# yangdongchao/Text-to-sound-Synthesis

Hardware: AMD Instinct MI355X
Metric: 10s clips/sec whole-node, 100-step Diffsound sample + VQ decode + vocoder (higher is better)
Workload: dtype f32 via 2-way fp16 split (3 MFMA passes, fp32 accumulate); 1 GPU; BASELINE configs[2]: full pipeline, batch 64 per GPU, 100 diffusion steps, codebook 256: CLIP text tower -> 19-layer denoiser -> SpecVQGAN decode -> MelGAN 22 kHz; global_batch=64, n_layer=19, parallelism=caption-sharded x1

## Files before the change

include/diffsound_hip.h:

```cpp
#ifndef DIFFSOUND_HIP_H
#define DIFFSOUND_HIP_H
#include <stdint.h>
#ifdef __cplusplus
extern "C" {
#endif

typedef void* ds_stream_t;

int ds_version(void);
const char* ds_last_error_string(void);

enum { DS_LOAD_DENSE = 0, DS_LOAD_CONV2D = 1, DS_LOAD_CONV1D = 2, DS_LOAD_CONVT1D = 3 };
enum { DS_PRO_NONE = 0, DS_PRO_AFFINE = 1, DS_PRO_AFFINE_SWISH = 2, DS_PRO_LRELU = 3 };
enum { DS_ACT_NONE = 0, DS_ACT_GELU2 = 1, DS_ACT_TANH = 2 };
enum { DS_STORE_ROW = 0, DS_STORE_BATCH_T = 1, DS_STORE_CONVT = 2, DS_STORE_ATTN = 3 };

typedef struct ds_gemm_desc {
    const float* A;
    const float* W;
    const float* bias;
    const float* R;
    float* C;
    int32_t M, N, K;
    int32_t lda, ldw, ldc, ldr;
    int32_t groups;
    int64_t a_gstride, w_gstride, c_gstride;
    int32_t loader, pro, act, store;
    const float* pro_scale;
    const float* pro_shift;
    int32_t rows_per_sample;
    int32_t Cin;
    int32_t H, Wd;
    int32_t up;
    int32_t taps, dil;
    int32_t ct_r, ct_p, ct_tin;
    int32_t f16_round;
    int64_t w3_plane;
    float out_scale;
    int32_t a_split, c_split;
    int64_t a_plane, c_plane;
    void* attn_kv;
    int32_t attn_heads, attn_nkey;
    int64_t attn_qplane;
} ds_gemm_desc;

int ds_gemm(const ds_gemm_desc* d, ds_stream_t stream);
void ds_gemm_force_tile(int cfg);
int ds_gemm_f16x2(const ds_gemm_desc* d, ds_stream_t stream);
int ds_gemm_f16x2_multi(const ds_gemm_desc* descs, int n, int cfg, ds_stream_t stream);
int ds_conv2d_f16x2(const ds_gemm_desc* d, ds_stream_t stream);
void ds_gemm_f16x2_force_tile(int cfg);
int ds_gemm_f16x2_auto_tile(int M, int N, int groups);
void ds_gemm_f16x2_set_balance_slots(int slots);
int ds_gemm_f16x2_plan(int cfg, int M, int N, int store, int* m_off, int* nbig, int* nsmall);

int ds_embed(const int64_t* tokens, const float* emb, const float* pos, float* out, int M, int L, int D,
             ds_stream_t stream);
int ds_adaln(const float* x, float* y, int M, int L, int D, const float* table, const int64_t* t,
             ds_stream_t stream);
int ds_layernorm(const float* x, float* y, int M, int D, const float* gamma, const float* beta,
                 ds_stream_t stream);
int ds_attention(const float* q, int ldq, const float* k, int ldk, const float* v, int ldv, float* o, int ldo,
                 int B, int heads, int Lq, int Lk, float scale, ds_stream_t stream);

int ds_attention_ex(const float* q, int ldq, const float* k, int ldk, const float* v, int ldv, float* o, int ldo,
                    int B, int heads, int Lq, int Lk, float scale, int causal, int f16_round, ds_stream_t stream);
int ds_attention_f16x2(const float* q, int ldq, const float* k, int ldk, const float* v, int ldv, float* o, int ldo,
                       int B, int heads, int Lq, int Lk, float scale, ds_stream_t stream);
int ds_adaln_split(const float* x, void* yh, int M, int L, int D, const float* table, const int64_t* t,
                   ds_stream_t stream);
int ds_layernorm_split(const float* x, void* yh, int M, int D, const float* gamma, const float* beta,
                       ds_stream_t stream);
int ds_attention_f16x2_split(const float* q, int ldq, const float* k, int ldk, const float* v, int ldv, void* oh,
                             int ldo, int B, int heads, int Lq, int Lk, float scale, ds_stream_t stream);
int ds_attn_nkey(int Lk);
int ds_attention_f16x2_ready(const void* qh, long long q_plane, const void* kv_img, void* oh, int ldo, int B, int heads,
                             int Lq, int Lk, float scale, ds_stream_t stream);
int ds_attn_pack_kv(const float* kv, int ld, int v_col, void* img, int B, int heads, int Lk, ds_stream_t stream);
int ds_embed_f16(const int64_t* tokens, const float* emb, const float* pos, float* out, int M, int L, int D,
                 ds_stream_t stream);
int ds_layernorm_f16(const float* x, float* y, int M, int D, const float* gamma, const float* beta,
                     ds_stream_t stream);
int ds_l2norm_rows_f16(const float* x, float* y, int M, int D, ds_stream_t stream);

// ... 243 lines not shown
```

text-to-sound-synthesis_amd/_lib.py:

```python
import ctypes as C
import os

import torch

_HERE = os.path.dirname(os.path.abspath(__file__))
LIB_PATH = os.environ.get("DIFFSOUND_LIB") or os.path.join(_HERE, "libdiffsound_hip.so")

LOAD_DENSE, LOAD_CONV2D, LOAD_CONV1D, LOAD_CONVT1D = 0, 1, 2, 3
PRO_NONE, PRO_AFFINE, PRO_AFFINE_SWISH, PRO_LRELU = 0, 1, 2, 3
ACT_NONE, ACT_GELU2, ACT_TANH = 0, 1, 2
STORE_ROW, STORE_BATCH_T, STORE_CONVT, STORE_ATTN = 0, 1, 2, 3
(LP_ADALN1, LP_W_QKV, LP_B_QKV, LP_W_PROJ1, LP_B_PROJ1, LP_ADALN2, LP_W_Q2, LP_B_Q2, LP_W_KV2, LP_B_KV2,
 LP_W_PROJ2, LP_B_PROJ2, LP_LN2_G, LP_LN2_B, LP_W_FC1, LP_B_FC1, LP_W_FC2, LP_B_FC2, LP_COUNT) = range(19)

_vp, _i32, _i64, _f = C.c_void_p, C.c_int32, C.c_int64, C.c_float


class GemmDesc(C.Structure):
    _fields_ = [("A", _vp), ("W", _vp), ("bias", _vp), ("R", _vp), ("C", _vp),
                ("M", _i32), ("N", _i32), ("K", _i32),
                ("lda", _i32), ("ldw", _i32), ("ldc", _i32), ("ldr", _i32),
                ("groups", _i32),
                ("a_gstride", _i64), ("w_gstride", _i64), ("c_gstride", _i64),
                ("loader", _i32), ("pro", _i32), ("act", _i32), ("store", _i32),
                ("pro_scale", _vp), ("pro_shift", _vp),
                ("rows_per_sample", _i32), ("Cin", _i32), ("H", _i32), ("Wd", _i32), ("up", _i32),
                ("taps", _i32), ("dil", _i32), ("ct_r", _i32), ("ct_p", _i32), ("ct_tin", _i32),
                ("f16_round", _i32), ("w3_plane", _i64), ("out_scale", _f),
                ("a_split", _i32), ("c_split", _i32), ("a_plane", _i64), ("c_plane", _i64),
                ("attn_kv", _vp), ("attn_heads", _i32), ("attn_nkey", _i32), ("attn_qplane", _i64)]


class DenoiserDesc(C.Structure):
    _fields_ = [("n_layer", _i32), ("n_embd", _i32), ("n_head", _i32), ("seq_len", _i32),
                ("cond_len", _i32), ("cond_dim", _i32), ("n_codes", _i32), ("n_steps", _i32),
                ("mlp_mult", _i32),
                ("tok_emb", _vp), ("pos_emb", _vp), ("lnf_g", _vp), ("lnf_b", _vp),
                ("w_logits", _vp), ("b_logits", _vp), ("sched", _vp)]


_PROTOS = {
    "ds_version": (C.c_int, []),
    "ds_last_error_string": (C.c_char_p, []),
    "ds_gemm": (C.c_int, [C.POINTER(GemmDesc), _vp]),
    "ds_gemm_force_tile": (None, [C.c_int]),
    "ds_gemm_f16x2": (C.c_int, [C.POINTER(GemmDesc), _vp]),
    "ds_conv2d_f16x2": (C.c_int, [C.POINTER(GemmDesc), _vp]),
    "ds_gemm_f16x2_multi": (C.c_int, [C.POINTER(GemmDesc), C.c_int, C.c_int, _vp]),
    "ds_gemm_f16x2_auto_tile": (C.c_int, [C.c_int, C.c_int, C.c_int]),
    "ds_gemm_f16x2_force_tile": (None, [C.c_int]),
    "ds_gemm_f16x2_set_balance_slots": (None, [C.c_int]),
    "ds_gemm_f16x2_plan": (C.c_int, [C.c_int, C.c_int, C.c_int, C.c_int, C.POINTER(C.c_int), C.POINTER(C.c_int), C.POINTER(C.c_int)]),
    "ds_denoiser_set_split_weights": (C.c_int, [_vp, C.c_int, C.POINTER(_vp), C.POINTER(_f), _vp, _f]),
    "ds_embed": (C.c_int, [_vp, _vp, _vp, _vp, C.c_int, C.c_int, C.c_int, _vp]),
    "ds_adaln": (C.c_int, [_vp, _vp, C.c_int, C.c_int, C.c_int, _vp, _vp, _vp]),
    "ds_layernorm": (C.c_int, [_vp, _vp, C.c_int, C.c_int, _vp, _vp, _vp]),
    "ds_attention": (C.c_int, [_vp, C.c_int, _vp, C.c_int, _vp, C.c_int, _vp, C.c_int,
                               C.c_int, C.c_int, C.c_int, C.c_int, _f, _vp]),
    "ds_attention_ex": (C.c_int, [_vp, C.c_int, _vp, C.c_int, _vp, C.c_int, _vp, C.c_int,
                                  C.c_int, C.c_int, C.c_int, C.c_int, _f, C.c_int, C.c_int, _vp]),
    "ds_attention_f16x2": (C.c_int, [_vp, C.c_int, _vp, C.c_int, _vp, C.c_int, _vp, C.c_int,
                                     C.c_int, C.c_int, C.c_int, C.c_int, _f, _vp]),
    "ds_adaln_split": (C.c_int, [_vp, _vp, C.c_int, C.c_int, C.c_int, _vp, _vp, _vp]),
    "ds_layernorm_split": (C.c_int, [_vp, _vp, C.c_int, C.c_int, _vp, _vp, _vp]),
    "ds_attention_f16x2_split": (C.c_int, [_vp, C.c_int, _vp, C.c_int, _vp, C.c_int, _vp, C.c_int,
                                           C.c_int, C.c_int, C.c_int, C.c_int, _f, _vp]),
    "ds_attn_nkey": (C.c_int, [C.c_int]),
    "ds_attention_f16x2_ready": (C.c_int, [_vp, _i64, _vp, _vp, C.c_int, C.c_int, C.c_int, C.c_int, C.c_int, _f, _vp]),
    "ds_attn_pack_kv": (C.c_int, [_vp, C.c_int, C.c_int, _vp, C.c_int, C.c_int, C.c_int, _vp]),
    "ds_embed_f16": (C.c_int, [_vp, _vp, _vp, _vp, C.c_int, C.c_int, C.c_int, _vp]),
    "ds_layernorm_f16": (C.c_int, [_vp, _vp, C.c_int, C.c_int, _vp, _vp, _vp]),
    "ds_l2norm_rows_f16": (C.c_int, [_vp, _vp, C.c_int, C.c_int, _vp]),
    "ds_sample_tail": (C.c_int, [_vp, _vp, _vp, _vp, _vp, _vp, _vp, _vp, _vp,
                                 C.c_int, C.c_int, C.c_int, C.c_int, C.c_int, _f, _vp]),
    "ds_sample_tail_ex": (C.c_int, [_vp, _vp, _vp, _vp, _vp, _vp, _vp, _vp, _vp,
                                    C.c_int, C.c_int, C.c_int, C.c_int, C.c_int, _f, C.c_int, _vp]),
    "ds_q_sample": (C.c_int, [_vp, _vp, _vp, _vp, _vp, C.c_int, C.c_int, C.c_int, C.c_int, _vp]),
    "ds_philox_uniforms": (C.c_int, [_vp, C.c_uint64, C.c_int, C.c_int, _vp, C.c_int, C.c_int, C.c_int, _vp]),
    "ds_sample_tail_rng": (C.c_int, [_vp, _vp, _vp, _vp, C.c_uint64, C.c_int, _vp, _vp, C.c_int, C.c_int, C.c_int, C.c_int,
                                     C.c_int, _f, C.c_int, _vp]),
    "ds_q_sample_rng": (C.c_int, [_vp, _vp, _vp, C.c_uint64, C.c_int, _vp, _vp, C.c_int, C.c_int, C.c_int, C.c_int, _vp]),
    "ds_vq_argmin": (C.c_int, [_vp, _vp, _vp, _vp, _vp, C.c_int, C.c_int, C.c_int, _vp]),
    "ds_loss_tail": (C.c_int, [_vp, _vp, _vp, _vp, _vp, _vp, _vp, _vp, _vp, C.c_int, C.c_int, C.c_int, C.c_int, _vp]),
# ... 258 lines not shown
```

text-to-sound-synthesis_amd/csrc/gemm_f16x2_ps.hip:

```cpp
#include <stdlib.h>

#include "common.h"


typedef _Float16 h8 __attribute__((ext_vector_type(8)));
typedef unsigned u32x4 __attribute__((ext_vector_type(4)));
typedef unsigned u32x2 __attribute__((ext_vector_type(2)));
typedef __attribute__((address_space(1))) const void* ds_gptr;
typedef __attribute__((address_space(3))) void* ds_lptr;

#define PS_HLD 32
#define PS_BM 288
#define PS_BN 256
#define PS_LEAD 6
#define PS_GM 4
#define PS_STAGE_BYTES (2 * 2 * (PS_BM + PS_BN) * PS_HLD * 2)
#define PS_EPI_BYTES (2 * 64 * (PS_BN + 4) * 4)
#ifndef PS_DIRECT_SPLIT
#define PS_DIRECT_SPLIT 1
#endif
#ifndef PS_DIRECT_QK
#define PS_DIRECT_QK 0
#endif
#define PS_LDS_BYTES (PS_EPI_BYTES > PS_STAGE_BYTES ? PS_EPI_BYTES : PS_STAGE_BYTES)
#define PS_SIG(q_) ((0x78 >> (2 * (q_))) & 3)

enum { PS_EPI_ROW = 0, PS_EPI_SPLIT = 1, PS_EPI_ATTN = 2 };

template <int EPI, bool NB16>
__global__ __launch_bounds__(512, 1) void ds_gemm_f16x2_ps_kernel(const GemmParams p) {
    extern __shared__ __attribute__((aligned(16))) unsigned char smem_raw[];
    constexpr int BM = PS_BM, BN = PS_BN, HLD = PS_HLD, LEAD = PS_LEAD;
    constexpr int APL = BM * HLD, BPL = BN * HLD, STAGE = 2 * (APL + BPL);
    _Float16* smem = (_Float16*)smem_raw;
    const int tid = threadIdx.x, lane = tid & 63, wave = tid >> 6, l31 = lane & 31, hh = lane >> 5;
    const int wr = wave >> 2, wc = wave & 3;
    const int L = p.rows_per_sample;
    const int tiles_n = p.N / BN, nblk = gridDim.x;
    int bid = blockIdx.x;
    {
        const int xcd = bid & 7, idx = bid >> 3, q = nblk >> 3, r = nblk & 7;
        bid = (xcd < r ? xcd * (q + 1) : r * (q + 1) + (xcd - r) * q) + idx;
    }
    int tm_, tn_;
    {
        const int tiles_m = p.M / L;
        const int per = PS_GM * tiles_n, grp = bid / per, first = grp * PS_GM;
        const int gsz = tiles_m - first < PS_GM ? tiles_m - first : PS_GM;
        const int in = bid - grp * per;
        tm_ = first + in % gsz;
        tn_ = in / gsz;
    }
    const int row_lo = tm_ * L;
    const int m0 = (row_lo >> 4) << 4, n0 = tn_ * BN;
    const int nk = p.K / 32;
    const _Float16* Ap = (const _Float16*)p.A;
    const _Float16* Wp = (const _Float16*)p.W;
    unsigned long long src[4][2], src8;
    int ldsoff[4][2], ldsoff8;
    const unsigned lane16 = lane * 16;
    const int rgsA = (p.M + 15) >> 4, rgsB = (p.N + 15) >> 4;
#define PS_BASE(dst_, ptr_)                                                                          \
    do {                                                                                             \
        const unsigned long long a_ = (unsigned long long)(ptr_);                                    \
        dst_ = ((unsigned long long)(unsigned)__builtin_amdgcn_readfirstlane((unsigned)(a_ >> 32)) << 32) | \
               (unsigned long long)(unsigned)__builtin_amdgcn_readfirstlane((unsigned)a_);           \
    } while (0)
#pragma unroll
    for (int ty = 0; ty < 4; ++ty)
#pragma unroll
        for (int k = 0; k < 2; ++k) {
            const int idx = 2 * wave + k, plane = idx >> 3, r = idx & 7;
            const bool isA = (ty == 0 || ty == 3);
            const int s = isA ? (ty == 3) : (ty == 2);
            const int gip = isA ? (r >> 2) * 8 + s * 4 + (r & 3)
                                : (r >> 1) * 4 + s * 2 + (r & 1);
            int rg = ((isA ? m0 : n0) >> 4) + gip;
            const int rgs = isA ? rgsA : rgsB;
            if (rg >= rgs) rg = rgs - 1;
            PS_BASE(src[ty][k], (isA ? Ap + plane * p.a_plane : Wp + plane * p.w3_plane) + (size_t)rg * nk * 512);
            ldsoff[ty][k] = __builtin_amdgcn_readfirstlane((isA ? plane * 18 + gip : 36 + plane * 16 + gip) * 1024);
        }
    {
        const int e = wave & 3, plane = e >> 1, gip = 16 + (e & 1);
        int rg = (m0 >> 4) + gip;
        if (rg >= rgsA) rg = rgsA - 1;
        PS_BASE(src8, Ap + plane * p.a_plane + (size_t)rg * nk * 512);
        ldsoff8 = __builtin_amdgcn_readfirstlane((plane * 18 + gip) * 1024);
    }
#define PS_ISSUE(tile_, ty_, buf_)                                                                   \
    do {                                                                                             \
        _Pragma("unroll") for (int k = 0; k < 2; ++k)                                                \
            __builtin_amdgcn_global_load_lds((ds_gptr)((const unsigned char*)(src[ty_][k] + (unsigned long long)(tile_) * 1024) + lane16), \
                                             (ds_lptr)(smem_raw + (buf_) * (STAGE * 2) + ldsoff[ty_][k]), 16, 0, 0); \
        if ((ty_) == 3)                                                                              \
            __builtin_amdgcn_global_load_lds((ds_gptr)((const unsigned char*)(src8 + (unsigned long long)(tile_) * 1024) + lane16), \
                                             (ds_lptr)(smem_raw + (buf_) * (STAGE * 2) + ldsoff8), 16, 0, 0); \
    } while (0)
#define PS_DMA_ASM(base_, lds_, stage_)                                                              \
    do {                                                                                             \
        asm volatile("s_add_u32 m0, %2, %3\n\ts_nop 0\n\tglobal_load_lds_dwordx4 %0, %1"            \
                     :: "v"(lane16), "s"(base_), "s"(lds_), "n"(stage_) : "memory", "scc", "m0");    \
        base_ += 1024;                                                                               \
    } while (0)
#define PS_ISSUE_LOOP(tq_, ty_, buf_)                                                                \
    do {                                                                                             \
        PS_DMA_ASM(cur[ty_][0], ldsabs[ty_][0], (buf_) * (STAGE * 2));                               \
        PS_DMA_ASM(cur[ty_][1], ldsabs[ty_][1], (buf_) * (STAGE * 2));                               \
        if ((ty_) == 3) PS_DMA_ASM(cur8, ldsabs8, (buf_) * (STAGE * 2));                             \
    } while (0)
#define PS_FENCE()                                                                                   \
    do { asm volatile("" ::: "memory"); __builtin_amdgcn_sched_barrier(0); } while (0)
#define PS_BAR()                                                                                     \
    do { PS_FENCE(); __builtin_amdgcn_s_barrier(); PS_FENCE(); } while (0)
#define PS_LBAR() PS_BAR()
    const int swz[2] = {((0 + hh) ^ ((l31 >> 2) & 3)) * 8, ((2 + hh) ^ ((l31 >> 2) & 3)) * 8};
    f32x16 acc[4][2], acc8;
    f32x4 acc9[2];
#pragma unroll
    for (int r = 0; r < 16; ++r) acc8[r] = 0.f;
#pragma unroll
    for (int tt = 0; tt < 2; ++tt) acc9[tt] = f32x4{0.f, 0.f, 0.f, 0.f};
#pragma unroll
    for (int i = 0; i < 4; ++i)
#pragma unroll
        for (int j = 0; j < 2; ++j)
#pragma unroll
            for (int r = 0; r < 16; ++r) acc[i][j][r] = 0.f;
    h8 a0[2][2], a1[2][2];
    h8 b0[2][2], b1[2][2];
    h8 e0[2], e1[2];
    h8 ea0, ea1, eb0[2], eb1[2];
    const int l15 = PS_SIG((lane >> 2) & 3) * 4 + (lane & 3);
    const int swzq = ((lane >> 4) ^ ((l15 >> 2) & 3)) * 8;
#define PS_READ_A(buf_, s_)                                                                          \
    do {                                                                                             \
        const _Float16* Ac = smem + (buf_) * STAGE + (wr * 128 + (s_) * 64 + l31) * HLD;             \
        _Pragma("unroll") for (int ks = 0; ks < 2; ++ks)                                             \
            _Pragma("unroll") for (int ib = 0; ib < 2; ++ib) {                                       \
                a0[ks][ib] = *(const h8*)(Ac + ib * 32 * HLD + swz[ks]);                             \
                a1[ks][ib] = *(const h8*)(Ac + APL + ib * 32 * HLD + swz[ks]);                       \
            }                                                                                        \
    } while (0)
#define PS_READ_E(buf_)                                                                              \
    do {                                                                                             \
        const _Float16* Ec = smem + (buf_) * STAGE + (256 + l31) * HLD;                              \
        _Pragma("unroll") for (int ks = 0; ks < 2; ++ks) {                                           \
            e0[ks] = *(const h8*)(Ec + swz[ks]);                                                     \
            e1[ks] = *(const h8*)(Ec + APL + swz[ks]);                                               \
        }                                                                                            \
    } while (0)
#define PS_READ_B(buf_, s_)                                                                          \
    do {                                                                                             \
        const _Float16* Bc = smem + (buf_) * STAGE + 2 * APL + (wc * 64 + (s_) * 32 + l31) * HLD;    \
        _Pragma("unroll") for (int ks = 0; ks < 2; ++ks) {                                           \
            b0[s_][ks] = *(const h8*)(Bc + swz[ks]);                                                 \
            b1[s_][ks] = *(const h8*)(Bc + BPL + swz[ks]);                                           \
        }                                                                                            \
    } while (0)
#define PS_QUAD(sa_, sb_)                                                                            \
    do {                                                                                             \
        _Pragma("unroll") for (int ks = 0; ks < 2; ++ks) {                                           \
            _Pragma("unroll") for (int ib = 0; ib < 2; ++ib)                                         \
                acc[2 * (sa_) + ib][sb_] = __builtin_amdgcn_mfma_f32_32x32x16_f16(b0[sb_][ks], a1[ks][ib], acc[2 * (sa_) + ib][sb_], 0, 0, 0); \
            _Pragma("unroll") for (int ib = 0; ib < 2; ++ib)                                         \
                acc[2 * (sa_) + ib][sb_] = __builtin_amdgcn_mfma_f32_32x32x16_f16(b1[sb_][ks], a0[ks][ib], acc[2 * (sa_) + ib][sb_], 0, 0, 0); \
            _Pragma("unroll") for (int ib = 0; ib < 2; ++ib)                                         \
                acc[2 * (sa_) + ib][sb_] = __builtin_amdgcn_mfma_f32_32x32x16_f16(b0[sb_][ks], a0[ks][ib], acc[2 * (sa_) + ib][sb_], 0, 0, 0); \
        }                                                                                            \
    } while (0)
#define PS_EXTRA(sb_)                                                                                \
    do {                                                                                             \
        _Pragma("unroll") for (int ks = 0; ks < 2; ++ks) {                                           \
            acc8 = __builtin_amdgcn_mfma_f32_32x32x16_f16(b0[sb_][ks], e1[ks], acc8, 0, 0, 0);       \
            acc8 = __builtin_amdgcn_mfma_f32_32x32x16_f16(b1[sb_][ks], e0[ks], acc8, 0, 0, 0);       \
            acc8 = __builtin_amdgcn_mfma_f32_32x32x16_f16(b0[sb_][ks], e0[ks], acc8, 0, 0, 0);       \
        }                                                                                            \
    } while (0)
#define PS_READ_EB16(buf_)                                                                           \
    do {                                                                                             \
        const _Float16* Bc = smem + (buf_) * STAGE + 2 * APL + ((2 * wc + wr) * 32 + l15) * HLD;     \
        _Pragma("unroll") for (int tt = 0; tt < 2; ++tt) {                                           \
            eb0[tt] = *(const h8*)(Bc + tt * 16 * HLD + swzq);                                       \
            eb1[tt] = *(const h8*)(Bc + BPL + tt * 16 * HLD + swzq);                                 \
        }                                                                                            \
    } while (0)
#define PS_READ_EA16(buf_)                                                                           \
    do {                                                                                             \
        const _Float16* Ec = smem + (buf_) * STAGE + (256 + l15) * HLD;                              \
        ea0 = *(const h8*)(Ec + swzq);                                                               \
        ea1 = *(const h8*)(Ec + APL + swzq);                                                         \
    } while (0)
#define PS_EXTRA16()                                                                                 \
    do {                                                                                             \
        _Pragma("unroll") for (int tt = 0; tt < 2; ++tt) {                                           \
            acc9[tt] = __builtin_amdgcn_mfma_f32_16x16x32_f16(eb0[tt], ea1, acc9[tt], 0, 0, 0);      \
            acc9[tt] = __builtin_amdgcn_mfma_f32_16x16x32_f16(eb1[tt], ea0, acc9[tt], 0, 0, 0);      \
            acc9[tt] = __builtin_amdgcn_mfma_f32_16x16x32_f16(eb0[tt], ea0, acc9[tt], 0, 0, 0);      \
        }                                                                                            \
    } while (0)
#define PS_PHASE(P, BUF)                                                                             \
    do {                                                                                             \
        if (P == 0) { PS_READ_A(BUF, 0); PS_READ_B(BUF, 0); }                                        \
        if (P == 1) { PS_READ_B(BUF, 1); if (NB16) PS_READ_EB16(BUF); }                              \
        if (P == 2) { PS_READ_A(BUF, 1); if (NB16) PS_READ_EA16(BUF); }                              \
        if (P == 3 && !NB16) PS_READ_E(BUF);                                                         \
        PS_FENCE();                                                                                  \
        {                                                                                            \
            constexpr int dq = (P) + LEAD;                                     \
            const int tq = t + (dq >> 2);                                                            \
            if (tq < nk) {                                                                           \
                PS_ISSUE_LOOP(tq, dq & 3, ((BUF) + (dq >> 2)) & 1);                                  \
                asm volatile("s_waitcnt vmcnt(9)" ::: "memory");    \
            } else {                                                                                 \
                asm volatile("s_waitcnt vmcnt(0)" ::: "memory");    \
            }                                                                                        \
        }                                                                                            \
        PS_LBAR();                                                                                   \
        __builtin_amdgcn_s_setprio(1);                                                               \
        if (P == 0) PS_QUAD(0, 0);                                                                   \
        if (P == 1) PS_QUAD(0, 1);                                                                   \
        if (P == 2) { PS_QUAD(1, 1); if (NB16) PS_EXTRA16(); }                                       \
        if (P == 3) { PS_QUAD(1, 0); if (!NB16) { if (wr == 0) PS_EXTRA(0); else PS_EXTRA(1); } }    \
        __builtin_amdgcn_s_setprio(0);                                                               \
        PS_LBAR();                                                                                   \
    } while (0)
#pragma unroll
    for (int q = 0; q < LEAD; ++q)
        if ((q >> 2) < nk) PS_ISSUE(q >> 2, q & 3, (q >> 2) & 1);
    if (4 * nk >= LEAD) asm volatile("s_waitcnt vmcnt(9)" ::: "memory");
    else asm volatile("s_waitcnt vmcnt(0)" ::: "memory");
    PS_BAR();
    if (wr == 1) PS_LBAR();
    unsigned long long cur[4][2], cur8 = src8 + 1024;
#pragma unroll
    for (int ty = 0; ty < 4; ++ty) {
        cur[ty][0] = src[ty][0] + (ty < 2 ? 2048 : 1024);
        cur[ty][1] = src[ty][1] + (ty < 2 ? 2048 : 1024);
    }
    const unsigned lds0 = __builtin_amdgcn_readfirstlane((unsigned)(size_t)(__attribute__((address_space(3))) unsigned char*)smem_raw);
    unsigned ldsabs[4][2], ldsabs8 = lds0 + ldsoff8;
#pragma unroll
    for (int ty = 0; ty < 4; ++ty) { ldsabs[ty][0] = lds0 + ldsoff[ty][0]; ldsabs[ty][1] = lds0 + ldsoff[ty][1]; }
    for (int t = 0; t < nk; t += 2) {
        PS_PHASE(0, 0); PS_PHASE(1, 0); PS_PHASE(2, 0); PS_PHASE(3, 0);
        ++t;
        PS_PHASE(0, 1); PS_PHASE(1, 1); PS_PHASE(2, 1); PS_PHASE(3, 1);
        --t;
    }
    if (wr == 0) PS_LBAR();
    asm volatile("s_waitcnt vmcnt(0)" ::: "memory");

    constexpr int WROW = 128, EROW0 = 256;
    constexpr bool HALF_TILE = false;
    const bool hasE = true;
    const int pos0 = 0, tile_rows = L;
#include "gemm_f16x2_ps_epilogue.inc"
}

#define PH_AROWS 144
#define PH_STAGE_BYTES (2 * (PH_AROWS + PS_BN) * PS_HLD * 2)
#define PH_LDS_BYTES (3 * PH_STAGE_BYTES > PS_EPI_BYTES ? 3 * PH_STAGE_BYTES : PS_EPI_BYTES)

template <int EPI>
__global__ __launch_bounds__(512, 1) void ds_gemm_f16x2_ph_kernel(const GemmParams p) {
    extern __shared__ __attribute__((aligned(16))) unsigned char smem_raw[];
    constexpr bool NB16 = true;
    constexpr int BN = PS_BN, HLD = PS_HLD;
    constexpr int APL = PH_AROWS * HLD, BPL = BN * HLD, STAGE = 2 * (APL + BPL);
    _Float16* smem = (_Float16*)smem_raw;
    const int tid = threadIdx.x, lane = tid & 63, wave = tid >> 6, l31 = lane & 31, hh = lane >> 5;
    const int wr = wave >> 2, wc = wave & 3;
    const int L = p.rows_per_sample;
    const int tiles_n = p.N / BN, nblk = gridDim.x;
    int bid = blockIdx.x;
    {
        const int xcd = bid & 7, idx = bid >> 3, q = nblk >> 3, r = nblk & 7;
        bid = (xcd < r ? xcd * (q + 1) : r * (q + 1) + (xcd - r) * q) + idx;
    }
    int th_, tn_;
    {
        const int tiles_m = 2 * (p.M / L);
        const int per = PS_GM * tiles_n, grp = bid / per, first = grp * PS_GM;
        const int gsz = tiles_m - first < PS_GM ? tiles_m - first : PS_GM;
        const int in = bid - grp * per;
        th_ = first + in % gsz;
        tn_ = in / gsz;
    }
    const int tm_ = th_ >> 1;
    const bool hasE = (th_ & 1) == 0;
// ... 135 lines not shown
        else { PH_QUAD(1); if (hasE) PH_EXTRA16(); }                                                 \
        __builtin_amdgcn_s_setprio(0);                                                               \
        PS_BAR();                                                                                    \
    } while (0)
    unsigned long long curA[2] = {srcA[0] + 2048, srcA[1] + 2048}, curE = srcE + 2048;
    unsigned long long curB[2][2] = {{srcB[0][0] + 2048, srcB[0][1] + 2048}, {srcB[1][0] + 2048, srcB[1][1] + 2048}};
    const unsigned lds0 = __builtin_amdgcn_readfirstlane((unsigned)(size_t)(__attribute__((address_space(3))) unsigned char*)smem_raw);
    const unsigned absA[2] = {lds0 + offA[0], lds0 + offA[1]}, absE = lds0 + offE;
    const unsigned absB[2][2] = {{lds0 + offB[0][0], lds0 + offB[0][1]}, {lds0 + offB[1][0], lds0 + offB[1][1]}};
#define PH_ISSUE_LOOP(half_, st_)                                                                    \
    do {                                                                                             \
        if ((half_) == 0) {                                                                          \
            PS_DMA_ASM(curA[0], absA[0], (st_) * (STAGE * 2)); PS_DMA_ASM(curA[1], absA[1], (st_) * (STAGE * 2)); \
            PS_DMA_ASM(curB[0][0], absB[0][0], (st_) * (STAGE * 2)); PS_DMA_ASM(curB[0][1], absB[0][1], (st_) * (STAGE * 2)); \
        } else {                                                                                     \
            PS_DMA_ASM(curB[1][0], absB[1][0], (st_) * (STAGE * 2)); PS_DMA_ASM(curB[1][1], absB[1][1], (st_) * (STAGE * 2)); \
            PS_DMA_ASM(curE, absE, (st_) * (STAGE * 2));                                             \
        }                                                                                            \
    } while (0)
    PH_ISSUE(0, 0, 0); PH_ISSUE(0, 1, 0);
    if (nk > 1) { PH_ISSUE(1, 0, 1); PH_ISSUE(1, 1, 1); asm volatile("s_waitcnt vmcnt(10)" ::: "memory"); }
    else asm volatile("s_waitcnt vmcnt(0)" ::: "memory");
    PS_BAR();
    if (wr == 1) PS_BAR();
    for (int t = 0; t < nk; t += 3) {
        { const int tt = t; PH_PHASE(0, 0); PH_PHASE(1, 0); }
        if (t + 1 < nk) { const int tt = t + 1; PH_PHASE(0, 1); PH_PHASE(1, 1); }
        if (t + 2 < nk) { const int tt = t + 2; PH_PHASE(0, 2); PH_PHASE(1, 2); }
    }
    if (wr == 0) PS_BAR();
    asm volatile("s_waitcnt vmcnt(0)" ::: "memory");
    constexpr int WROW = 64, EROW0 = 128;
    constexpr bool HALF_TILE = true;
#include "gemm_f16x2_ps_epilogue.inc"
}

static bool ps_serves(const GemmParams& p, bool half) {
    const int L = p.rows_per_sample;
    if (!p.a_split || L <= 0 || L > PS_BM - 15 || L <= 240 || p.M % L != 0) return false;
    if (half && L != PS_BM - 16) return false;
    if (p.N % PS_BN != 0 || p.K % 64 != 0 || p.lda != p.K || p.ldw != p.K) return false;
    if (((uintptr_t)p.bias & 15) != 0) return false;
    if (p.store == DS_STORE_ROW && !p.c_split) {
        if (((p.N | p.ldc | p.ldr) & 3) != 0 || (((uintptr_t)p.C | (uintptr_t)p.R) & 15) != 0) return false;
    } else if (p.store == DS_STORE_ROW) {
        if (p.R) return false;
    } else if (p.store == DS_STORE_ATTN) {
        if (p.row_off != 0 || p.attn_heads * 64 % PS_BN != 0) return false;
    } else {
        return false;
    }
    return true;
}

int ds_gemm_f16x2_ps_choice(long B, long N, bool half_ok) {
    const long tf = B * (N / PS_BN), th = 2 * tf;
    const double ef = (double)tf / (double)(((tf + 255) / 256) * 256);
    const double eh = half_ok ? 0.92 * (double)th / (double)(((th + 255) / 256) * 256) : 0.0;
    if (ef < 0.65 && eh < 0.65) return 0;
    return ef >= eh ? 1 : 2;
}

bool ds_gemm_f16x2_ps_applies(const GemmParams& p, bool need_full_grid) {
    if (!ps_serves(p, false)) return false;
    return !need_full_grid || ds_gemm_f16x2_ps_choice(p.M / p.rows_per_sample, p.N, false) == 1;
}
bool ds_gemm_f16x2_ph_applies(const GemmParams& p) { return ps_serves(p, true); }
int ds_gemm_f16x2_ps_pick(const GemmParams& p) {
    if (!ps_serves(p, false)) return 0;
    return ds_gemm_f16x2_ps_choice(p.M / p.rows_per_sample, p.N, ps_serves(p, true));
}

template <int EPI, bool NB16>
static int launch_ps(const GemmParams& p, hipStream_t s) {
    static DsOnce attr_set;
    if (attr_set.need()) {
        hipError_t e = hipFuncSetAttribute((const void*)ds_gemm_f16x2_ps_kernel<EPI, NB16>,
                                           hipFuncAttributeMaxDynamicSharedMemorySize, PS_LDS_BYTES);
        if (e != hipSuccess) {
            ds_set_error("gemm_f16x2_ps: hipFuncSetAttribute: %s", hipGetErrorString(e));
            return -2;
        }
        attr_set.done();
    }
    const int tiles = (p.M / p.rows_per_sample) * (p.N / PS_BN);
    hipLaunchKernelGGL((ds_gemm_f16x2_ps_kernel<EPI, NB16>), dim3(tiles), dim3(512), PS_LDS_BYTES, s, p);
    DS_CHECK_LAUNCH();
    return 0;
}

int ds_launch_gemm_f16x2_ps(const GemmParams& p, hipStream_t s) {
    const bool nb16 = p.rows_per_sample == PS_BM - 16;
    if (p.store == DS_STORE_ATTN) return nb16 ? launch_ps<PS_EPI_ATTN, true>(p, s) : launch_ps<PS_EPI_ATTN, false>(p, s);
    if (p.c_split) return nb16 ? launch_ps<PS_EPI_SPLIT, true>(p, s) : launch_ps<PS_EPI_SPLIT, false>(p, s);
    return nb16 ? launch_ps<PS_EPI_ROW, true>(p, s) : launch_ps<PS_EPI_ROW, false>(p, s);
}

template <int EPI>
static int launch_ph(const GemmParams& p, hipStream_t s) {
    static DsOnce attr_set;
    if (attr_set.need()) {
        hipError_t e = hipFuncSetAttribute((const void*)ds_gemm_f16x2_ph_kernel<EPI>,
                                           hipFuncAttributeMaxDynamicSharedMemorySize, PH_LDS_BYTES);
        if (e != hipSuccess) {
            ds_set_error("gemm_f16x2_ph: hipFuncSetAttribute: %s", hipGetErrorString(e));
            return -2;
        }
        attr_set.done();
    }
    const int tiles = 2 * (p.M / p.rows_per_sample) * (p.N / PS_BN);
    hipLaunchKernelGGL((ds_gemm_f16x2_ph_kernel<EPI>), dim3(tiles), dim3(512), PH_LDS_BYTES, s, p);
    DS_CHECK_LAUNCH();
    return 0;
}

int ds_launch_gemm_f16x2_ph(const GemmParams& p, hipStream_t s) {
    if (p.store == DS_STORE_ATTN) return launch_ph<PS_EPI_ATTN>(p, s);
    if (p.c_split) return launch_ph<PS_EPI_SPLIT>(p, s);
    return launch_ph<PS_EPI_ROW>(p, s);
// ... 2 lines not shown
```

text-to-sound-synthesis_amd/csrc/gemm_f16x2_ps_epilogue.inc:

```
    int tid_e = tid;
    asm volatile("" : "+v"(tid_e));
    const int l31e = tid_e & 31, hhe = (tid_e >> 5) & 1, wre = tid_e >> 8, wce = (tid_e >> 6) & 3;
    const int off = row_lo - m0;
    int vhi = off + tile_rows;
    if (vhi > p.M - m0) vhi = p.M - m0;
    const float osc = p.out_scale;
    constexpr bool ALLV = NB16;
    const int qe = (tid_e >> 4) & 3, ne = tid_e & 15;
    const int cb0 = (wce * 2 + 0) * 32, cb1 = (wce * 2 + 1) * 32, cb9 = (wce * 2 + wre) * 32;
    const int cq = 4 * hhe, cq9 = NB16 ? 4 * PS_SIG(qe) : cq;
    const int r9 = NB16 ? 4 * PS_SIG(ne >> 2) + (ne & 3) : l31e;
    const bool hasb = p.bias != nullptr;
    const float* bsrc = (hasb ? p.bias : (const float*)p.W) + n0;
#define PS_BIAS4(col_) (hasb ? *(const f32x4*)(bsrc + (col_)) : f32x4{0.f, 0.f, 0.f, 0.f})
#define PS_BIAS1(col_) (hasb ? bsrc[col_] : 0.f)
#define PS_FIN(x_, b_, GELU, t_)                                                                     \
    do {                                                                                             \
        t_ = (x_) * osc + (b_);                                                                      \
        if (GELU) t_ = ds_gelu2_fast(t_);                                                            \
    } while (0)
    constexpr int ELD = BN + 4, EBUF = 64 * ELD;
#define PS_TROW(S, rs_) ((S) < 4 ? ((rs_) >> 5) * WROW + (S) * 32 + ((rs_) & 31) : EROW0 + (rs_))
#define PS_STEP_QUADS(S, STORE4)                                                                     \
    do {                                                                                             \
// ... 275 lines not shown
                        PS_VT_UNIT(g, r0, cl, bvt[3], x);                                    \
                        u32x4 vh, vl;                                                                \
                        PS_UNZIP(x, vh, vl);                                                         \
                        *(u32x4*)dst = vh;                                                           \
                        *(u32x4*)(dst + pln) = vl;                                                   \
                    } else {                                                                         \
                        _Pragma("unroll") for (int e = 0; e < 8; ++e)                                \
                            if (r0 + e >= lo - G0 && r0 + e < hi - G0) {                             \
                                float t1;                                                            \
                                if (gelu) PS_FIN(PS_VT_W(g, r0 + e, cl), bvt[3], true, t1);   \
                                else PS_FIN(PS_VT_W(g, r0 + e, cl), bvt[3], false, t1);       \
                                const unsigned x1 = ds_split_pack(t1);                               \
                                dst[e] = __builtin_bit_cast(_Float16, (unsigned short)(x1 & 0xffffu)); \
                                dst[pln + e] = __builtin_bit_cast(_Float16, (unsigned short)(x1 >> 16)); \
                            }                                                                        \
                    }                                                                                \
                }                                                                                    \
            }                                                                                        \
        }                                                                                            \
    } while (0)
        if (EPI == PS_EPI_ATTN && which == 2) {
            const float bvt[4] = {PS_BIAS1(tid_e >> 2), PS_BIAS1((tid_e >> 2) + 128), PS_BIAS1(tid_e >> 1),
                                  PS_BIAS1(tid_e & (BN - 1))};
            if constexpr (!HALF_TILE) {
                PS_VT_STEP(0); PS_VT_STEP(1); PS_VT_STEP(2); PS_VT_STEP(3); PS_VT_STEP(4);
            } else {
                PS_VT_STEP(0); PS_VT_STEP(1);
                if (hasE) PS_VT_STEP(4);
            }
        } else {
            constexpr bool DIRECT = EPI == PS_EPI_SPLIT ? PS_DIRECT_SPLIT : PS_DIRECT_QK;
            if constexpr (DIRECT) {
                PS_DIRECT_BIAS();
                if constexpr (!HALF_TILE) {
                    PS_DIRECT_STEP(0); PS_DIRECT_STEP(1); PS_DIRECT_STEP(2); PS_DIRECT_STEP(3); PS_DIRECT_STEP(4);
                } else {
                    PS_DIRECT_STEP(0); PS_DIRECT_STEP(1);
                    if (hasE) PS_DIRECT_STEP(4);
                }
            } else {
                float bias8[8];
                *(f32x4*)bias8 = PS_BIAS4((tid_e & 31) * 8);
                *(f32x4*)(bias8 + 4) = PS_BIAS4((tid_e & 31) * 8 + 4);
                if constexpr (!HALF_TILE) {
                    PS_SPLIT_STEP(0); PS_SPLIT_STEP(1); PS_SPLIT_STEP(2); PS_SPLIT_STEP(3); PS_SPLIT_STEP(4);
                } else {
                    PS_SPLIT_STEP(0); PS_SPLIT_STEP(1);
                    if (hasE) PS_SPLIT_STEP(4);
                }
            }
        }
    }
#undef PS_TROW
#undef PS_STEP_QUADS
#undef PS_BIAS4
#undef PS_BIAS1
#undef PS_FIN
#undef PS_ST_RAW
#undef PS_FIN_SPLIT8
#undef PS_VT_UNIT
#undef PS_DIRECT_BIAS
#undef PS_ROW_STEP
#undef PS_ROW_ALL
#undef PS_ROW_STAGE
#undef PS_ROW_STORE
#undef PS_ROW_LOAD
// ... 15 lines not shown
```

Before: 22.80 clips/s.

## Make PS GEMM kernel persistent and prefetch next tile during split epilogue

Turns the full-tile PS GEMM kernel into a persistent kernel whose grid is capped at the CU count (rounded to a multiple of 8). Each workgroup loops over tiles via a shared tile-mapping helper. For the direct-split NB16 epilogue, it computes the next tile's source bases and issues the prologue loads before the epilogue stores, so the next mainloop starts with data in flight (vmcnt raised to 45). This aims to hide the per-tile fill latency and launch tail, at the cost of more register pressure and more complex vmcnt accounting. It also exposes force-grid and tile-of hooks for testing.

```diff
diff --git a/include/diffsound_hip.h b/include/diffsound_hip.h
--- a/include/diffsound_hip.h
+++ b/include/diffsound_hip.h
@@ -50,6 +50,8 @@
 int ds_gemm_f16x2_multi(const ds_gemm_desc* descs, int n, int cfg, ds_stream_t stream);
 int ds_conv2d_f16x2(const ds_gemm_desc* d, ds_stream_t stream);
 void ds_gemm_f16x2_force_tile(int cfg);
+void ds_gemm_f16x2_ps_force_grid(int g);
+void ds_gemm_f16x2_ps_tile_of(int wg, int step, int grid, int tiles_m, int tiles_n, int* tm, int* tn);
 int ds_gemm_f16x2_auto_tile(int M, int N, int groups);
 void ds_gemm_f16x2_set_balance_slots(int slots);
 int ds_gemm_f16x2_plan(int cfg, int M, int N, int store, int* m_off, int* nbig, int* nsmall);
diff --git a/text-to-sound-synthesis_amd/_lib.py b/text-to-sound-synthesis_amd/_lib.py
--- a/text-to-sound-synthesis_amd/_lib.py
+++ b/text-to-sound-synthesis_amd/_lib.py
@@ -49,6 +49,8 @@
     "ds_gemm_f16x2_multi": (C.c_int, [C.POINTER(GemmDesc), C.c_int, C.c_int, _vp]),
     "ds_gemm_f16x2_auto_tile": (C.c_int, [C.c_int, C.c_int, C.c_int]),
     "ds_gemm_f16x2_force_tile": (None, [C.c_int]),
+    "ds_gemm_f16x2_ps_force_grid": (None, [C.c_int]),
+    "ds_gemm_f16x2_ps_tile_of": (None, [C.c_int, C.c_int, C.c_int, C.c_int, C.c_int, C.POINTER(C.c_int), C.POINTER(C.c_int)]),
     "ds_gemm_f16x2_set_balance_slots": (None, [C.c_int]),
     "ds_gemm_f16x2_plan": (C.c_int, [C.c_int, C.c_int, C.c_int, C.c_int, C.POINTER(C.c_int), C.POINTER(C.c_int), C.POINTER(C.c_int)]),
     "ds_denoiser_set_split_weights": (C.c_int, [_vp, C.c_int, C.POINTER(_vp), C.POINTER(_f), _vp, _f]),
diff --git a/text-to-sound-synthesis_amd/csrc/gemm_f16x2_ps.hip b/text-to-sound-synthesis_amd/csrc/gemm_f16x2_ps.hip
--- a/text-to-sound-synthesis_amd/csrc/gemm_f16x2_ps.hip
+++ b/text-to-sound-synthesis_amd/csrc/gemm_f16x2_ps.hip
@@ -27,38 +27,37 @@
 
 enum { PS_EPI_ROW = 0, PS_EPI_SPLIT = 1, PS_EPI_ATTN = 2 };
 
+__host__ __device__ static inline void ps_tile_of(int wg, int step, int grid, int tiles_m, int tiles_n, int* tm, int* tn) {
+    const int nblk = tiles_m * tiles_n;
+    int bid = wg + step * grid;
+    {
+        const int xcd = bid & 7, idx = bid >> 3, q = nblk >> 3, r = nblk & 7;
+        bid = (xcd < r ? xcd * (q + 1) : r * (q + 1) + (xcd - r) * q) + idx;
+    }
+    const int per = PS_GM * tiles_n, grp = bid / per, first = grp * PS_GM;
+    const int gsz = tiles_m - first < PS_GM ? tiles_m - first : PS_GM;
+    const int in = bid - grp * per;
+    *tm = first + in % gsz;
+    *tn = in / gsz;
+}
+extern "C" void ds_gemm_f16x2_ps_tile_of(int wg, int step, int grid, int tiles_m, int tiles_n, int* tm, int* tn) {
+    ps_tile_of(wg, step, grid, tiles_m, tiles_n, tm, tn);
+}
+
 template <int EPI, bool NB16>
 __global__ __launch_bounds__(512, 1) void ds_gemm_f16x2_ps_kernel(const GemmParams p) {
     extern __shared__ __attribute__((aligned(16))) unsigned char smem_raw[];
     constexpr int BM = PS_BM, BN = PS_BN, HLD = PS_HLD, LEAD = PS_LEAD;
     constexpr int APL = BM * HLD, BPL = BN * HLD, STAGE = 2 * (APL + BPL);
+    constexpr bool REFILL = EPI == PS_EPI_SPLIT && PS_DIRECT_SPLIT && NB16;
     _Float16* smem = (_Float16*)smem_raw;
-    const int tid = threadIdx.x, lane = tid & 63, wave = tid >> 6, l31 = lane & 31, hh = lane >> 5;
-    const int wr = wave >> 2, wc = wave & 3;
     const int L = p.rows_per_sample;
-    const int tiles_n = p.N / BN, nblk = gridDim.x;
-    int bid = blockIdx.x;
-    {
-        const int xcd = bid & 7, idx = bid >> 3, q = nblk >> 3, r = nblk & 7;
-        bid = (xcd < r ? xcd * (q + 1) : r * (q + 1) + (xcd - r) * q) + idx;
-    }
-    int tm_, tn_;
-    {
-        const int tiles_m = p.M / L;
-        const int per = PS_GM * tiles_n, grp = bid / per, first = grp * PS_GM;
-        const int gsz = tiles_m - first < PS_GM ? tiles_m - first : PS_GM;
-        const int in = bid - grp * per;
-        tm_ = first + in % gsz;
-        tn_ = in / gsz;
-    }
-    const int row_lo = tm_ * L;
-    const int m0 = (row_lo >> 4) << 4, n0 = tn_ * BN;
+    const int tiles_n = p.N / BN, tiles_m = p.M / L, tiles = tiles_m * tiles_n;
+    const int wg = blockIdx.x, grid = gridDim.x;
     const int nk = p.K / 32;
     const _Float16* Ap = (const _Float16*)p.A;
     const _Float16* Wp = (const _Float16*)p.W;
     unsigned long long src[4][2], src8;
-    int ldsoff[4][2], ldsoff8;
-    const unsigned lane16 = lane * 16;
     const int rgsA = (p.M + 15) >> 4, rgsB = (p.N + 15) >> 4;
 #define PS_BASE(dst_, ptr_)                                                                          \
     do {                                                                                             \
@@ -66,28 +65,30 @@
         dst_ = ((unsigned long long)(unsigned)__builtin_amdgcn_readfirstlane((unsigned)(a_ >> 32)) << 32) | \
                (unsigned long long)(unsigned)__builtin_amdgcn_readfirstlane((unsigned)a_);           \
     } while (0)
-#pragma unroll
-    for (int ty = 0; ty < 4; ++ty)
-#pragma unroll
-        for (int k = 0; k < 2; ++k) {
-            const int idx = 2 * wave + k, plane = idx >> 3, r = idx & 7;
-            const bool isA = (ty == 0 || ty == 3);
-            const int s = isA ? (ty == 3) : (ty == 2);
-            const int gip = isA ? (r >> 2) * 8 + s * 4 + (r & 3)
-                                : (r >> 1) * 4 + s * 2 + (r & 1);
-            int rg = ((isA ? m0 : n0) >> 4) + gip;
-            const int rgs = isA ? rgsA : rgsB;
-            if (rg >= rgs) rg = rgs - 1;
-            PS_BASE(src[ty][k], (isA ? Ap + plane * p.a_plane : Wp + plane * p.w3_plane) + (size_t)rg * nk * 512);
-            ldsoff[ty][k] = __builtin_amdgcn_readfirstlane((isA ? plane * 18 + gip : 36 + plane * 16 + gip) * 1024);
-        }
-    {
-        const int e = wave & 3, plane = e >> 1, gip = 16 + (e & 1);
-        int rg = (m0 >> 4) + gip;
-        if (rg >= rgsA) rg = rgsA - 1;
-        PS_BASE(src8, Ap + plane * p.a_plane + (size_t)rg * nk * 512);
-        ldsoff8 = __builtin_amdgcn_readfirstlane((plane * 18 + gip) * 1024);
-    }
+#define PS_XFER(w_, ty_, k_)                                                                          \
+    const int idx = 2 * (w_) + (k_), plane = idx >> 3, r = idx & 7;                                  \
+    const bool isA = ((ty_) == 0 || (ty_) == 3);                                                     \
+    const int s = isA ? ((ty_) == 3) : ((ty_) == 2);                                                 \
+    const int gip = isA ? (r >> 2) * 8 + s * 4 + (r & 3)        \
+                        : (r >> 1) * 4 + s * 2 + (r & 1)
+#define PS_TILE_BASES(w_, m0_, n0_)                                                                  \
+    do {                                                                                             \
+        _Pragma("unroll") for (int ty = 0; ty < 4; ++ty)                                             \
+            _Pragma("unroll") for (int k = 0; k < 2; ++k) {                                          \
+                PS_XFER(w_, ty, k);                                                                  \
+                int rg = ((isA ? (m0_) : (n0_)) >> 4) + gip;                                         \
+                const int rgs = isA ? rgsA : rgsB;                                                   \
+                if (rg >= rgs) rg = rgs - 1;                        \
+                PS_BASE(src[ty][k], (isA ? Ap + plane * p.a_plane : Wp + plane * p.w3_plane) + (size_t)rg * nk * 512); \
+            }                                                                                        \
+        {    \
+            const int e = (w_) & 3, plane = e >> 1, gip = 16 + (e & 1);                              \
+            int rg = ((m0_) >> 4) + gip;                                                             \
+            if (rg >= rgsA) rg = rgsA - 1;                                                           \
+            PS_BASE(src8, Ap + plane * p.a_plane + (size_t)rg * nk * 512);                           \
+        }                                                                                            \
+    } while (0)
+    int step = 0, tm_ = 0, tn_ = 0;
 #define PS_ISSUE(tile_, ty_, buf_)                                                                   \
     do {                                                                                             \
         _Pragma("unroll") for (int k = 0; k < 2; ++k)                                                \
@@ -114,25 +115,12 @@
 #define PS_BAR()                                                                                     \
     do { PS_FENCE(); __builtin_amdgcn_s_barrier(); PS_FENCE(); } while (0)
 #define PS_LBAR() PS_BAR()
-    const int swz[2] = {((0 + hh) ^ ((l31 >> 2) & 3)) * 8, ((2 + hh) ^ ((l31 >> 2) & 3)) * 8};
     f32x16 acc[4][2], acc8;
     f32x4 acc9[2];
-#pragma unroll
-    for (int r = 0; r < 16; ++r) acc8[r] = 0.f;
-#pragma unroll
-    for (int tt = 0; tt < 2; ++tt) acc9[tt] = f32x4{0.f, 0.f, 0.f, 0.f};
-#pragma unroll
-    for (int i = 0; i < 4; ++i)
-#pragma unroll
-        for (int j = 0; j < 2; ++j)
-#pragma unroll
-            for (int r = 0; r < 16; ++r) acc[i][j][r] = 0.f;
     h8 a0[2][2], a1[2][2];
     h8 b0[2][2], b1[2][2];
     h8 e0[2], e1[2];
     h8 ea0, ea1, eb0[2], eb1[2];
-    const int l15 = PS_SIG((lane >> 2) & 3) * 4 + (lane & 3);
-    const int swzq = ((lane >> 4) ^ ((l15 >> 2) & 3)) * 8;
 #define PS_READ_A(buf_, s_)                                                                          \
     do {                                                                                             \
         const _Float16* Ac = smem + (buf_) * STAGE + (wr * 128 + (s_) * 64 + l31) * HLD;             \
@@ -199,7 +187,7 @@
             acc9[tt] = __builtin_amdgcn_mfma_f32_16x16x32_f16(eb0[tt], ea0, acc9[tt], 0, 0, 0);      \
         }                                                                                            \
     } while (0)
-#define PS_PHASE(P, BUF)                                                                             \
+#define PS_PHASE_W(P, BUF, W)                                                                        \
     do {                                                                                             \
         if (P == 0) { PS_READ_A(BUF, 0); PS_READ_B(BUF, 0); }                                        \
         if (P == 1) { PS_READ_B(BUF, 1); if (NB16) PS_READ_EB16(BUF); }                              \
@@ -211,7 +199,7 @@
             const int tq = t + (dq >> 2);                                                            \
             if (tq < nk) {                                                                           \
                 PS_ISSUE_LOOP(tq, dq & 3, ((BUF) + (dq >> 2)) & 1);                                  \
-                asm volatile("s_waitcnt vmcnt(9)" ::: "memory");    \
+                asm volatile("s_waitcnt vmcnt(" #W ")" ::: "memory");    \
             } else {                                                                                 \
                 asm volatile("s_waitcnt vmcnt(0)" ::: "memory");    \
             }                                                                                        \
@@ -225,37 +213,121 @@
         __builtin_amdgcn_s_setprio(0);                                                               \
         PS_LBAR();                                                                                   \
     } while (0)
-#pragma unroll
-    for (int q = 0; q < LEAD; ++q)
-        if ((q >> 2) < nk) PS_ISSUE(q >> 2, q & 3, (q >> 2) & 1);
-    if (4 * nk >= LEAD) asm volatile("s_waitcnt vmcnt(9)" ::: "memory");
-    else asm volatile("s_waitcnt vmcnt(0)" ::: "memory");
-    PS_BAR();
-    if (wr == 1) PS_LBAR();
-    unsigned long long cur[4][2], cur8 = src8 + 1024;
-#pragma unroll
-    for (int ty = 0; ty < 4; ++ty) {
-        cur[ty][0] = src[ty][0] + (ty < 2 ? 2048 : 1024);
-        cur[ty][1] = src[ty][1] + (ty < 2 ? 2048 : 1024);
-    }
-    const unsigned lds0 = __builtin_amdgcn_readfirstlane((unsigned)(size_t)(__attribute__((address_space(3))) unsigned char*)smem_raw);
-    unsigned ldsabs[4][2], ldsabs8 = lds0 + ldsoff8;
-#pragma unroll
-    for (int ty = 0; ty < 4; ++ty) { ldsabs[ty][0] = lds0 + ldsoff[ty][0]; ldsabs[ty][1] = lds0 + ldsoff[ty][1]; }
-    for (int t = 0; t < nk; t += 2) {
-        PS_PHASE(0, 0); PS_PHASE(1, 0); PS_PHASE(2, 0); PS_PHASE(3, 0);
-        ++t;
-        PS_PHASE(0, 1); PS_PHASE(1, 1); PS_PHASE(2, 1); PS_PHASE(3, 1);
-        --t;
-    }
-    if (wr == 0) PS_LBAR();
-    asm volatile("s_waitcnt vmcnt(0)" ::: "memory");
-
-    constexpr int WROW = 128, EROW0 = 256;
-    constexpr bool HALF_TILE = false;
-    const bool hasE = true;
-    const int pos0 = 0, tile_rows = L;
+#define PS_PHASE(P, BUF) PS_PHASE_W(P, BUF, 9)
+#define PS_FILL()                                                                                    \
+    do {                                                                                             \
+        _Pragma("unroll") for (int q = 0; q < LEAD; ++q)                                             \
+            if ((q >> 2) < nk) PS_ISSUE(q >> 2, q & 3, (q >> 2) & 1);                                \
+    } while (0)
+#define PS_REFILL_W 45
+    static_assert(PS_REFILL_W == 9 + 36 && PS_REFILL_W < 64, "vmcnt is a 6-bit counter");
+    bool filled = false;
+    for (;;) {
+        int tid = threadIdx.x;
+        asm volatile("" : "+v"(tid));
+        const int lane = tid & 63, wave = tid >> 6, l31 = lane & 31, hh = lane >> 5;
+        const int wr = wave >> 2, wc = wave & 3;
+        const int wave_s = __builtin_amdgcn_readfirstlane(wave);
+        const unsigned lane16 = lane * 16;
+        const int swz[2] = {((0 + hh) ^ ((l31 >> 2) & 3)) * 8, ((2 + hh) ^ ((l31 >> 2) & 3)) * 8};
+        const int l15 = PS_SIG((lane >> 2) & 3) * 4 + (lane & 3);
+        const int swzq = ((lane >> 4) ^ ((l15 >> 2) & 3)) * 8;
+        int ldsoff[4][2], ldsoff8;
+#pragma unroll
+        for (int ty = 0; ty < 4; ++ty)
+#pragma unroll
+            for (int k = 0; k < 2; ++k) {
+                PS_XFER(wave_s, ty, k);
+                ldsoff[ty][k] = (isA ? plane * 18 + gip : 36 + plane * 16 + gip) * 1024;
+            }
+        ldsoff8 = (((wave_s & 3) >> 1) * 18 + 16 + (wave_s & 1)) * 1024;
+        const unsigned lds0 = __builtin_amdgcn_readfirstlane((unsigned)(size_t)(__attribute__((address_space(3))) unsigned char*)smem_raw);
+        unsigned ldsabs[4][2], ldsabs8 = lds0 + ldsoff8;
+#pragma unroll
+        for (int ty = 0; ty < 4; ++ty) { ldsabs[ty][0] = lds0 + ldsoff[ty][0]; ldsabs[ty][1] = lds0 + ldsoff[ty][1]; }
+        if (!(REFILL && filled)) {
+            ps_tile_of(wg, step, grid, tiles_m, tiles_n, &tm_, &tn_);
+            PS_TILE_BASES(wave_s, ((tm_ * L) >> 4) << 4, tn_ * BN);
+        }
+        const int row_lo = tm_ * L;
+        const int m0 = (row_lo >> 4) << 4, n0 = tn_ * BN;
+        const bool more = wg + (step + 1) * grid < tiles;
+        int tm_nx = 0, tn_nx = 0;
+#pragma unroll
+        for (int r = 0; r < 16; ++r) acc8[r] = 0.f;
+#pragma unroll
+        for (int tt = 0; tt < 2; ++tt) acc9[tt] = f32x4{0.f, 0.f, 0.f, 0.f};
+#pragma unroll
+        for (int i = 0; i < 4; ++i)
+#pragma unroll
+            for (int j = 0; j < 2; ++j)
+#pragma unroll
+                for (int r = 0; r < 16; ++r) acc[i][j][r] = 0.f;
+        if (REFILL && filled) {
+            asm volatile("s_waitcnt vmcnt(45)" ::: "memory");
+        } else {
+            PS_FILL();
+            if (4 * nk >= LEAD) asm volatile("s_waitcnt vmcnt(9)" ::: "memory");
+            else asm volatile("s_waitcnt vmcnt(0)" ::: "memory");
+        }
+        PS_BAR();
+        if (wr == 1) PS_LBAR();
+        unsigned long long cur[4][2], cur8 = src8 + 1024;
+#pragma unroll
+        for (int ty = 0; ty < 4; ++ty) {
+            cur[ty][0] = src[ty][0] + (ty < 2 ? 2048 : 1024);
+            cur[ty][1] = src[ty][1] + (ty < 2 ? 2048 : 1024);
+        }
+        int t = 0;
+        if (REFILL && filled) {
+            PS_PHASE_W(0, 0, 45); PS_PHASE_W(1, 0, 45); PS_PHASE_W(2, 0, 45); PS_PHASE_W(3, 0, 45);
+            ++t;
+            PS_PHASE(0, 1); PS_PHASE(1, 1); PS_PHASE(2, 1); PS_PHASE(3, 1);
+            ++t;
+        }
+        for (; t < nk; t += 2) {
+            PS_PHASE(0, 0); PS_PHASE(1, 0); PS_PHASE(2, 0); PS_PHASE(3, 0);
+            ++t;
+            PS_PHASE(0, 1); PS_PHASE(1, 1); PS_PHASE(2, 1); PS_PHASE(3, 1);
+            --t;
+        }
+        if (wr == 0) PS_LBAR();
+        asm volatile("s_waitcnt vmcnt(0)" ::: "memory");
+        filled = false;
+
+#define PS_REFILL_HOOK(bq_)                                                                          \
+    do {                                                                                             \
+         \
+        if (REFILL && more) {                                                                        \
+            ps_tile_of(wg, step + 1, grid, tiles_m, tiles_n, &tm_nx, &tn_nx);                        \
+            PS_TILE_BASES(wave_s, ((tm_nx * L) >> 4) << 4, tn_nx * BN);                              \
+        }                                                                                            \
+         \
+         \
+        if (REFILL)                                                                                  \
+            _Pragma("unroll") for (int i_ = 0; i_ < 3; ++i_)                                         \
+                _Pragma("unroll") for (int j_ = 0; j_ < 4; ++j_) asm volatile("" : "+v"((bq_)[i_][j_])); \
+        if (REFILL && more) {                                                                        \
+            PS_FILL();                                                                               \
+            filled = true;                                                                           \
+        }                                                                                            \
+    } while (0)
+        constexpr int WROW = 128, EROW0 = 256;
+        constexpr bool HALF_TILE = false;
+        const bool hasE = true;
+        const int pos0 = 0, tile_rows = L;
 #include "gemm_f16x2_ps_epilogue.inc"
+#undef PS_REFILL_HOOK
+        if (!more) break;
+        ++step;
+        if (REFILL) {
+            tm_ = tm_nx;
+            tn_ = tn_nx;
+        } else {
+            asm volatile("s_waitcnt lgkmcnt(0)" ::: "memory");
+            PS_BAR();
+        }
+    }
 }
 
 #define PH_AROWS 144
@@ -457,7 +529,9 @@
     asm volatile("s_waitcnt vmcnt(0)" ::: "memory");
     constexpr int WROW = 64, EROW0 = 128;
     constexpr bool HALF_TILE = true;
+#define PS_REFILL_HOOK(bq_) do { } while (0)
 #include "gemm_f16x2_ps_epilogue.inc"
+#undef PS_REFILL_HOOK
 }
 
 static bool ps_serves(const GemmParams& p, bool half) {
@@ -496,6 +570,26 @@
     return ds_gemm_f16x2_ps_choice(p.M / p.rows_per_sample, p.N, ps_serves(p, true));
 }
 
+static int g_force_grid = 0;
+extern "C" void ds_gemm_f16x2_ps_force_grid(int g) { g_force_grid = g; }
+static int ps_grid_cap() {
+    static DsOnce once;
+    static std::atomic<int> cap[64];
+    const int d = DsOnce::dev();
+    if (once.need()) {
+        hipDeviceProp_t prop;
+        hipError_t e = hipGetDeviceProperties(&prop, d);
+        if (e != hipSuccess) {
+            ds_set_error("gemm_f16x2_ps: hipGetDeviceProperties: %s", hipGetErrorString(e));
+            return -1;
+        }
+        const int g = prop.multiProcessorCount & ~7;
+        cap[d].store(g < 8 ? 8 : g, std::memory_order_relaxed);
+        once.done();
+    }
+    return cap[d].load(std::memory_order_relaxed);
+}
+
 template <int EPI, bool NB16>
 static int launch_ps(const GemmParams& p, hipStream_t s) {
     static DsOnce attr_set;
@@ -509,7 +603,9 @@
         attr_set.done();
     }
     const int tiles = (p.M / p.rows_per_sample) * (p.N / PS_BN);
-    hipLaunchKernelGGL((ds_gemm_f16x2_ps_kernel<EPI, NB16>), dim3(tiles), dim3(512), PS_LDS_BYTES, s, p);
+    const int cap = g_force_grid > 0 ? g_force_grid : ps_grid_cap();
+    if (cap <= 0) return -2;
+    hipLaunchKernelGGL((ds_gemm_f16x2_ps_kernel<EPI, NB16>), dim3(tiles < cap ? tiles : cap), dim3(512), PS_LDS_BYTES, s, p);
     DS_CHECK_LAUNCH();
     return 0;
 }
diff --git a/text-to-sound-synthesis_amd/csrc/gemm_f16x2_ps_epilogue.inc b/text-to-sound-synthesis_amd/csrc/gemm_f16x2_ps_epilogue.inc
--- a/text-to-sound-synthesis_amd/csrc/gemm_f16x2_ps_epilogue.inc
+++ b/text-to-sound-synthesis_amd/csrc/gemm_f16x2_ps_epilogue.inc
@@ -331,6 +331,7 @@
             constexpr bool DIRECT = EPI == PS_EPI_SPLIT ? PS_DIRECT_SPLIT : PS_DIRECT_QK;
             if constexpr (DIRECT) {
                 PS_DIRECT_BIAS();
+                PS_REFILL_HOOK(bqd);
                 if constexpr (!HALF_TILE) {
                     PS_DIRECT_STEP(0); PS_DIRECT_STEP(1); PS_DIRECT_STEP(2); PS_DIRECT_STEP(3); PS_DIRECT_STEP(4);
                 } else {
```

Result: no change. 22.94 clips/s, median of 6 (+0.6%).
